# numericalEFT/FeynmanDiagram.jl

Measured on AMD Instinct MI355X. Metric: graph-evaluations/sec, higher is better.
Workload: dtype f64

## Files before the change

feynmandiagram.jl_amd/capi.py:

```python
from __future__ import annotations

import ctypes as C
import os
from typing import Optional

import numpy as np

from .nodetable import NodeTable

_HERE = os.path.dirname(os.path.abspath(__file__))
LIB_PATH = os.environ.get("FDG_LIBRARY") or os.path.join(_HERE, "lib", "libfdg.so")
KERNEL_CACHE = os.path.join(_HERE, "kernel_cache")

FDG_OK = 0
FDG_E_INVALID, FDG_E_UNSUPPORTED, FDG_E_NO_DEVICE, FDG_E_NOMEM, FDG_E_JIT, FDG_E_INTERNAL = -1, -2, -3, -4, -5, -6
FDG_SPEC_DEFAULT, FDG_SPEC_KEEP_SOURCE, FDG_SPEC_FAST_MATH, FDG_SPEC_ISA, FDG_SPEC_AUTOTUNE = 0, 1, 2, 4, 8
FDG_DT_F64, FDG_DT_F32, FDG_DT_C64, FDG_DT_C32 = 0, 1, 2, 3
DTYPES = {"Float64": FDG_DT_F64, "Float32": FDG_DT_F32, "ComplexF64": FDG_DT_C64, "ComplexF32": FDG_DT_C32}
FDG_SPEC_ROW_MAJOR_COMPANION = 16
FDG_ASSOC_STATIC, FDG_ASSOC_INTERP = 0, 1
FDG_TILE_SAMPLES = 64

EXPORTS = [
    "fdg_last_error", "fdg_version", "fdg_graph_create", "fdg_graph_destroy", "fdg_graph_query",
    "fdg_graph_emit_source", "fdg_free", "fdg_graph_specialize", "fdg_eval_device", "fdg_eval",
    "fdg_accumulate_device", "fdg_fill_uniform_device", "fdg_copy_device", "fdg_read_device", "fdg_clock_probe_device", "fdg_graph_specialize_typed", "fdg_eval_device_typed", "fdg_graph_create_complex_view", "fdg_isa_check_hazards", "fdg_graph_release_device", "fdg_powi",
    "fdg_eval_strided", "fdg_graph_coop_program", "fdg_graph_set_opt_params", "fdg_graph_opt_program", "fdg_graph_set_schedule_groups", "fdg_leaf_eval_device", "fdg_leaf_eval_device_tiled",
    "fdg_comm_unique_id", "fdg_comm_create", "fdg_comm_destroy", "fdg_reduce_device",
    "fdg_graph_specialize_fused", "fdg_mc_eval_device", "fdg_mc_accumulate_device", "fdg_graph_mc_program",
    "fdg_graph_kernel_info",
    "fdg_eval_device_tiled", "fdg_accumulate_device_tiled", "fdg_fill_uniform_device_tiled", "fdg_graph_set_association",
    "fdg_batch_alloc", "fdg_batch_free", "fdg_graph_pool_program", "fdg_batch_alloc_pair", "fdg_graph_set_option", "fdg_graph_get_option", "fdg_set_default_option", "fdg_get_default_option", "fdg_selftest_pair_search",
    "fdg_repack_tile_major", "fdg_unpack_tile_major",
    "fdg_accumulate_device_binned", "fdg_mc_accumulate_device_binned",
    "fdg_accumulate_device_moments", "fdg_mc_accumulate_device_moments",
    "fdg_vegas_sample_device", "fdg_accumulate_device_vegas", "fdg_mc_accumulate_device_vegas", "fdg_vegas_refine",
    "fdg_vegas_sample_device_discrete", "fdg_accumulate_device_vegas_binned", "fdg_mc_accumulate_device_vegas_binned",
    "fdg_vegas_refine_discrete",
    "fdg_vegas_sample_device_polar", "fdg_sincos",
    "fdg_matsubara_phase", "fdg_accumulate_device_matsubara", "fdg_mc_accumulate_device_matsubara",
    "fdg_vegas_sample_device_grouped", "fdg_accumulate_device_grouped", "fdg_mc_accumulate_device_grouped",
    "fdg_accumulate_device_observables", "fdg_mc_accumulate_device_observables",
    "fdg_accumulate_device_freq_observables", "fdg_mc_accumulate_device_freq_observables",
    "fdg_vegas_sample_device_strat", "fdg_accumulate_device_strat", "fdg_mc_accumulate_device_strat", "fdg_strat_allocate",
    "fdg_vegas_sample_device_strat_grouped", "fdg_accumulate_device_strat_grouped", "fdg_mc_accumulate_device_strat_grouped",
    "fdg_strat_allocate_cols",
    "fdg_chain_propose_device", "fdg_chain_step_device", "fdg_mc_chain_step_device", "fdg_chain_reduce_device",
# ... 142 lines not shown
    L.fdg_free.argtypes = [vp]
    L.fdg_free.restype = None
    L.fdg_graph_specialize.argtypes = [vp, C.c_char_p, C.c_uint]
    L.fdg_eval_device.argtypes = [vp, dp, i64, i64, dp, i64, i64, i64, vp]
    L.fdg_eval.argtypes = [vp, dp, dp, i64]
    L.fdg_graph_set_association.argtypes = [vp, C.c_int]
    L.fdg_batch_alloc.argtypes = [C.c_size_t, C.c_size_t, C.POINTER(vp)]
    L.fdg_batch_free.argtypes = [vp]
    L.fdg_graph_set_option.argtypes = [vp, C.c_char_p, C.c_char_p]
    L.fdg_graph_get_option.argtypes = [vp, C.c_char_p]
    L.fdg_graph_get_option.restype = C.c_char_p
    L.fdg_set_default_option.argtypes = [C.c_char_p, C.c_char_p]
    L.fdg_get_default_option.argtypes = [C.c_char_p]
    L.fdg_get_default_option.restype = C.c_char_p
    L.fdg_selftest_pair_search.argtypes = [C.c_uint64, C.c_uint32, C.c_uint32, C.POINTER(C.c_uint32)]
    L.fdg_batch_alloc_pair.argtypes = [vp, C.c_int64, C.c_size_t, C.c_uint, C.POINTER(vp), C.POINTER(vp), C.POINTER(BatchPairInfo)]
    L.fdg_eval_device_tiled.argtypes = [vp, dp, i64, i64, i64, dp, i64, i64, i64, i64, vp]
    L.fdg_accumulate_device_tiled.argtypes = [vp, dp, i64, i64, i64, dp, dp, i64, vp]
    L.fdg_fill_uniform_device_tiled.argtypes = [dp, i64, u32, i64, i64, i64, u64, u64, vp]
    L.fdg_eval_strided.argtypes = [vp, dp, i64, i64, dp, i64, i64, i64]
    L.fdg_accumulate_device.argtypes = [vp, dp, i64, i64, dp, dp, i64, vp]
    L.fdg_fill_uniform_device.argtypes = [dp, i64, u32, i64, i64, u64, u64, vp]
    L.fdg_copy_device.argtypes = [dp, dp, i64, vp]
    L.fdg_read_device.argtypes = [dp, i64, dp, vp]
    L.fdg_repack_tile_major.argtypes = [dp, i64, i64, dp, i64, C.c_uint32, vp]
    L.fdg_unpack_tile_major.argtypes = [dp, dp, i64, i64, i64, C.c_uint32, vp]
    L.fdg_clock_probe_device.argtypes = [C.c_double, vp, vp]
    L.fdg_graph_specialize_typed.argtypes = [vp, C.c_int, C.c_char_p, C.c_uint]
    L.fdg_eval_device_typed.argtypes = [vp, C.c_int, vp, i64, i64, vp, i64, i64, i64, vp]
    L.fdg_graph_create_complex_view.argtypes = [vp, C.POINTER(vp)]
# ... 1693 lines not shown
```

feynmandiagram.jl_amd/csrc/fdg_internal.h:

```cpp
#pragma once
#include <cstdint>
#include <mutex>
#include <string>
#include <vector>

#include "../../include/fdg.h"
#include "fdg_knobs.h"

namespace fdg {

constexpr uint32_t SP_LDS = 0u, SP_MEM = 1u, SP_LEAF = 2u;
constexpr uint32_t LOC_FAC = 1u << 29;
constexpr uint32_t LOC_IDX_MASK = (1u << 29) - 1u;
inline uint32_t mkloc(uint32_t space, uint32_t idx) { return (space << 30) | idx; }

constexpr uint32_t UOP_SUM = 0, UOP_PROD = 1, UOP_POW = 2, UOP_ROOT = 3, UOP_LEAF = 4, UOP_END = 5, UOP_PRODI = 6;

struct Lowered {
  uint32_t L = 0, N = 0, R = 0, E = 0;
  std::vector<uint8_t> op;
  std::vector<int32_t> power;
  std::vector<uint32_t> off, idx;
  std::vector<double> fac;
  std::vector<uint32_t> root_slot;
// ... 37 lines not shown
  void *s2 = nullptr, *ev_t[2] = {nullptr, nullptr}, *ev_k[2] = {nullptr, nullptr}, *ev_in = nullptr;
  uint64_t last_use = 0;
};

struct fdg_launch_cfg {
  bool no_rl = false, no_fused_acc = false, no_pool = false, pool_no_acc = false, no_streaming = false, no_w2 = false, no_coop = false, no_rm = false;
  bool transpose_narrow = false;
  uint32_t root_scratch_min = 16;
  uint64_t root_scratch_mb = 256;
  int waves_per_cu = 0;
  int oversub = 0;
  long mem_waves = -1;
  long mem_oversub = 1;
  double mem_ratio = 2.5;
  int tile_claim = -1;
  uint64_t sm_chunk_bytes = 1ull << 29;
  long long eval_chunk = 0, mc_chunk = 0;
};

enum { FDG_K_EVAL = 0, FDG_K_NT, FDG_K_W2, FDG_K_ACC, FDG_K_ACC_NT, FDG_K_RM, FDG_K_RM_ACC, FDG_K_RL, FDG_K_RL_ACC, FDG_K_COOP, FDG_K_POOL, FDG_K_EVAL_CL, FDG_K_NT_CL, FDG_K_COUNT };
static const char *const FDG_ISA_KERNEL[FDG_K_COUNT] = {"fdg_isa_eval", "fdg_isa_eval_nt", "fdg_isa_eval_w2", "fdg_isa_eval_acc", "fdg_isa_eval_acc_nt",
    "fdg_isa_eval_rm", "fdg_isa_eval_rm_acc", "fdg_isa_eval_rl", "fdg_isa_eval_rl_acc", "fdg_isa_eval_coop", "fdg_isa_eval_pool", "fdg_isa_eval_cl", "fdg_isa_eval_nt_cl"};
inline const char *fdg_isa_suffix(int k) { return FDG_ISA_KERNEL[k] + sizeof("fdg_isa_eval") - 1; }
struct fdg_isa_kernel {
  bool present = false;
  void *fn = nullptr;
  uint32_t vgpr = 0, lds_bytes = 0, mem_slots = 0, threads = 64;
};

struct fdg_graph {
// ... 11 lines not shown
  unsigned spec_flags = 0;
  uint32_t spec_vgpr = 0, spec_lds = 0, spec_scratch = 0;
  std::mutex mu;
  void *d_code = nullptr;
  void *d_root_live = nullptr;
  void *d_ws = nullptr;
  size_t ws_bytes = 0;
  void *module = nullptr;
  void *fn_eval_sm = nullptr, *fn_eval_gen = nullptr;
  bool isa = false;
  bool isa_fma = false;
  fdg_isa_kernel kern[FDG_K_COUNT];
  uint64_t st_valu[3] = {0, 0, 0};
  uint32_t st_ld_leaf[3] = {0, 0, 0}, st_panel[3] = {0, 0, 0}, st_lds[3] = {0, 0, 0};
  const char *last_kernel = "";
  uint32_t claim_run = 0;
  uint32_t last_launch = 0;
  uint32_t rm_bufs = 0;
  uint64_t rl_valu = 0;
  bool coop_enabled = false;
  uint32_t coop_panel_wg = 0;
  uint32_t pool_panel_wg = 0, pool_fetch = 0, pool_unit = 1;
  uint64_t pool_valu = 0;
  std::vector<char> alt_code;
  void *alt_module = nullptr, *fn_alt_sm = nullptr, *fn_alt_gen = nullptr;
  std::vector<char> fused_code;
  void *fused_module = nullptr, *fn_fused = nullptr;
  std::vector<char> typed_code[4];
  void *typed_module[4] = {nullptr, nullptr, nullptr, nullptr}, *fn_typed[4] = {nullptr, nullptr, nullptr, nullptr};
  fdg_graph *cx_twin = nullptr;
  bool cx_twin_tried = false;
// ... 84 lines not shown
```

feynmandiagram.jl_amd/csrc/fdg_isa.cpp:

```cpp
#include <algorithm>
#include <cctype>
#include <cinttypes>
#include <cmath>
#include <cstdio>
#include <cstdlib>
#include <cstring>
#include <map>
#include <sstream>

#include "fdg_opt.h"

namespace fdg {
int isa_claim_run_log2() {
  const char *e = fdg::knob("FDG_ISA_CLAIM_RUN");
  const long tiles = e ? std::atol(e) : 4;
  int r = 0;
  while (r < 6 && (1l << (r + 1)) <= tiles) ++r;
  return r;
}
namespace {

constexpr int V_LANE8 = 1, V_LEAFOFF = 2, V_ROOTOFF = 3, V_TMP = 4, V_BASE = 6;
constexpr int S_LEAF = 4, S_SS = 6, S_LS = 8, S_ROOT = 10, S_RS = 12, S_RK = 14, S_WS = 16, S_B = 18, S_NWG = 20;
constexpr int S_TILE = 22, S_NTILES = 23, S_LT = 24, S_RT = 26, S_PANEL = 28, S_LS8 = 30, S_RK8 = 32, S_A = 34,
              S_T = 36, S_C = 38, S_X = 40;
constexpr int S_WGT = 44;
constexpr int S_RTS = 44;
constexpr int S_LTS = 46;
constexpr int S_LP = 48;
constexpr int S_DELTA = 50;
constexpr int N_DELTA = 6;
constexpr int S_POOL = S_DELTA + 2 * N_DELTA;
constexpr int N_POOL = 20;
// ... 466 lines not shown
  const bool use_ldexp = fdg::knob("FDG_ISA_NO_LDEXP") == nullptr;
  const bool dbg_novalu = dbg && std::strstr(dbg, "novalu");
  const bool dbg_nopanel = dbg && std::strstr(dbg, "nopanel");
  const bool dbg_norecv = dbg && std::strstr(dbg, "norecv");
  const bool dbg_nofetch = dbg && std::strstr(dbg, "nopoolfetch");
  const bool dbg_noacc = dbg && std::strstr(dbg, "noacc");
  const bool dbg_nohead = dbg && std::strstr(dbg, "nohead");
  bool in_head = true;
  int tile_run = 0;
  if (dbg && std::strstr(dbg, "chunk") && !cs) tile_run = std::max(0, std::min(9, std::atoi(std::strstr(dbg, "chunk") + 5)));
  const bool tile_xcd = dbg && std::strstr(dbg, "xcd") && !cs && !tile_run;
  int tile_rot = 0;
  if (dbg && std::strstr(dbg, "rot") && !cs && !tile_run && !tile_xcd) tile_rot = std::max(0, std::atoi(std::strstr(dbg, "rot") + 3));
  const int S_ROTB = S_POOL + 2 * (N_POOL - 1), S_ROTS = S_ROTB + 1;
  const bool claim = claim_tiles && W == 1 && !cs && !accumulate && !rm_bufs && !rl && prog.mc_n_k == 0 && prog.mc_n_t == 0 && !tile_run && !tile_xcd && !tile_rot;
  const int claim_run = claim ? isa_claim_run_log2() : 0;
  const int S_CLAIM = S_POOL + 2 * (N_POOL - 1);
  uint64_t claim_seq = 0;
  E.vm_slack = (dbg && std::strstr(dbg, "noackwait") && !accumulate) ? p.R : 0;
  E.no_vm_wait = dbg && std::strstr(dbg, "novmwait");
  if (cs) E.ins("v_and_b32_e32 v0, 63, v0");
  E.ins("s_load_dwordx8 s[4:11], s[0:1], 0x0");
  E.ins("s_load_dwordx8 s[12:19], s[0:1], 0x20");
  E.ins("s_load_dwordx2 s[20:21], s[0:1], 0x40");
  if (accumulate) E.ins("s_load_dwordx2 " + S2(S_WGT) + ", s[0:1], 0x48");
  const uint32_t n_k = prog.mc_n_k;
  const bool mc = n_k > 0 || prog.mc_n_t > 0;
  const bool tm_imm = dbg && std::strstr(dbg, "tmimm") && !mc && !rm_bufs && !rl && !cs && W == 1;
  int64_t tm_base = -1;
  const int tile_arg = mc ? 0x80 : 0x50;
  E.ins("s_load_dwordx2 " + S2(S_LTS) + ", s[0:1], " + hex32((uint32_t)tile_arg));
  if (!accumulate) E.ins("s_load_dwordx2 " + S2(S_RTS) + ", s[0:1], " + hex32((uint32_t)tile_arg + 8));
  if (claim) E.ins("s_load_dwordx2 " + S2(S_CLAIM) + ", s[0:1], " + hex32((uint32_t)tile_arg + 16));
  if (mc) {
    E.ins("s_load_dwordx4 s[" + std::to_string(S_LEAF2) + ":" + std::to_string(S_LEAF2 + 3) + "], s[0:1], 0x50");
    E.ins("s_load_dwordx8 s[" + std::to_string(S_PARAM) + ":" + std::to_string(S_PARAM + 7) + "], s[0:1], 0x60");
  }
  E.ins("s_waitcnt lgkmcnt(0)");
  uint64_t w_seq = 0;
  const uint32_t acc0 = V_BASE + RW * std::max<uint32_t>(prog.n_reg_used, 1);
  const bool aa = accumulate && prog.params.acc_in_agpr;
  const uint32_t A0 = RW * prog.n_acc_used;
  const uint32_t acc_pairs_v = accumulate ? (aa ? 3 : p.R + 2) : 0;
  const uint32_t wgt0 = aa ? acc0 : acc0 + 2 * p.R;
  auto vpair = [&](uint32_t b) { return "v[" + std::to_string(b) + ":" + std::to_string(b + 1) + "]"; };
  auto vacc = [&](uint32_t k) { return vpair(acc0 + 2 * k); };
  const std::string vwgt = vpair(wgt0), vtmp = vpair(wgt0 + 2), vtmp2 = vpair(wgt0 + 4);
  auto acc_to_tmp2 = [&](uint32_t k) {
// ... 123 lines not shown
  E.ins("s_add_u32 " + S(S_X) + ", " + S(S_B) + ", " + std::to_string((1 << TSH) - 1));
  E.ins("s_addc_u32 " + S(S_X + 1) + ", " + S(S_B + 1) + ", 0");
  E.ins("s_lshr_b64 " + S2(S_X) + ", " + S2(S_X) + ", " + std::to_string(TSH));
  E.ins("s_mov_b32 " + S(S_NTILES) + ", " + S(S_X));
  if (tile_run) E.ins("s_lshl_b32 " + S(S_TILE) + ", s2, " + std::to_string(tile_run));
  else if (tile_xcd) {
    E.ins("s_and_b32 " + S(S_X) + ", s2, 7");
    E.ins("s_add_u32 " + S(S_T) + ", " + S(S_NTILES) + ", 7");
    E.ins("s_lshr_b32 " + S(S_T) + ", " + S(S_T) + ", 3");
    E.ins("s_mul_i32 " + S(S_A) + ", " + S(S_X) + ", " + S(S_T));
    E.ins("s_lshr_b32 " + S(S_A + 1) + ", s2, 3");
    E.ins("s_add_u32 " + S(S_TILE) + ", " + S(S_A) + ", " + S(S_A + 1));
    E.ins("s_add_u32 " + S(S_A) + ", " + S(S_A) + ", " + S(S_T));
    E.ins("s_min_u32 " + S(S_NTILES) + ", " + S(S_A) + ", " + S(S_NTILES));
  }
  else if (claim_run) E.ins("s_lshl_b32 " + S(S_TILE) + ", s2, " + std::to_string(claim_run));
  else {
    E.ins("s_mov_b32 " + S(S_TILE) + ", s2");
    if (tile_rot) { E.ins("s_mov_b32 " + S(S_ROTB) + ", 0"); E.ins("s_mov_b32 " + S(S_ROTS) + ", s2"); }
  }
  E.ins("s_mul_i32 " + S(S_X) + ", s2, " + hex32(cs ? cs->panel_wg_bytes : panel_bytes_per_wave));
  E.ins("s_mul_hi_u32 " + S(S_X + 1) + ", s2, " + hex32(cs ? cs->panel_wg_bytes : panel_bytes_per_wave));
  E.ins("s_add_u32 " + S(S_PANEL) + ", " + S(S_WS) + ", " + S(S_X));
  E.ins("s_addc_u32 " + S(S_PANEL + 1) + ", " + S(S_WS + 1) + ", " + S(S_X + 1));
  if (cs && cs->panel_prefix_bytes) {
    E.ins("s_add_u32 " + S(S_PANEL) + ", " + S(S_PANEL) + ", " + hex32(cs->panel_prefix_bytes));
    E.ins("s_addc_u32 " + S(S_PANEL + 1) + ", " + S(S_PANEL + 1) + ", 0");
  }
  std::map<uint32_t, int> panel_base;
  if (!mc) {
    std::map<uint32_t, uint64_t> hist;
// ... 8 lines not shown
    std::sort(v.begin(), v.end(), [](const auto &x, const auto &y) { return x.first > y.first || (x.first == y.first && x.second < y.second); });
    for (size_t i = 0; i < v.size() && pool.size() + i < (size_t)(N_POOL - (claim ? 1 : 0)); ++i) {
      const int r = S_POOL + 2 * (int)(pool.size() + i);
      panel_base[v[i].second] = r;
      E.ins("s_add_u32 " + S(r) + ", " + S(S_PANEL) + ", " + hex32(v[i].second * 8192u));
      E.ins("s_addc_u32 " + S(r + 1) + ", " + S(S_PANEL + 1) + ", 0");
    }
  }
  E.ins("s_cmp_ge_u32 " + S(S_TILE) + ", " + S(S_NTILES));
  E.ins("s_cbranch_scc0 .Ltile" + sfx);
  E.ins("s_endpgm");
  os << ".Ltile" << sfx << ":\n";
  if (cs && cs->slack) E.ins("s_mov_b32 " + S(S_DELTA + 7) + ", " + S(S_DELTA + 6));
  const int v_claim = (int)(tmp0 + 2 * n_tmp_pairs);
  if (claim) {
    if (claim_run) {
      E.ins("s_and_b32 " + S(S_X) + ", " + S(S_TILE) + ", " + std::to_string((1 << claim_run) - 1));
      E.ins("s_cbranch_scc1 .Lheld" + sfx);
    }
    E.ins("s_mov_b64 exec, 1");
    E.ins("v_mov_b32_e32 " + V(V_TMP) + ", 1");
    E.ins("global_atomic_add " + V(v_claim) + ", " + V(V_LANE8) + ", " + V(V_TMP) + ", " + S2(S_CLAIM) + " sc0");
    if (claim_run) os << ".Lheld" << sfx << ":\n";
    claim_seq = ++E.vm_issued;
  }
  E.ins("s_mov_b32 " + S(S_X + 1) + ", 0");
  E.ins("s_mov_b32 " + S(S_X) + ", " + S(S_TILE));
  E.ins("s_lshl_b64 " + S2(S_X) + ", " + S2(S_X) + ", " + std::to_string(TSH));
  if (W == 1) {
    E.ins("s_sub_u32 " + S(S_T) + ", " + S(S_B) + ", " + S(S_X));
    E.ins("s_subb_u32 " + S(S_T + 1) + ", " + S(S_B + 1) + ", " + S(S_X + 1));
    E.ins("s_cmp_lg_u32 " + S(S_T + 1) + ", 0");
    E.ins("s_cselect_b32 " + S(S_T) + ", 64, " + S(S_T));
    E.ins("s_min_u32 " + S(S_T) + ", " + S(S_T) + ", 64");
    E.ins("s_bfm_b64 " + S2(S_A) + ", " + S(S_T) + ", 0");
    E.ins("s_cmp_ge_u32 " + S(S_T) + ", 64");
    E.ins("s_cselect_b64 exec, -1, " + S2(S_A));
  }
// ... 553 lines not shown
    E.ins("s_cbranch_scc1 .Lrun" + sfx);
    E.ins("s_lshl_b32 " + S(S_X) + ", " + S(S_NWG) + ", " + std::to_string(tile_run));
    E.ins("s_add_u32 " + S(S_TILE) + ", " + S(S_TILE) + ", " + S(S_X));
    E.ins("s_sub_u32 " + S(S_TILE) + ", " + S(S_TILE) + ", " + std::to_string(1 << tile_run));
    os << ".Lrun" << sfx << ":\n";
  } else if (tile_xcd) {
    E.ins("s_lshr_b32 " + S(S_X) + ", " + S(S_NWG) + ", 3");
    E.ins("s_add_u32 " + S(S_TILE) + ", " + S(S_TILE) + ", " + S(S_X));
  } else if (tile_rot) {
    E.ins("s_add_u32 " + S(S_ROTB) + ", " + S(S_ROTB) + ", " + S(S_NWG));
    E.ins("s_add_u32 " + S(S_ROTS) + ", " + S(S_ROTS) + ", " + std::to_string(tile_rot));
    E.ins("s_sub_u32 " + S(S_X) + ", " + S(S_NWG) + ", 1");
    E.ins("s_and_b32 " + S(S_ROTS) + ", " + S(S_ROTS) + ", " + S(S_X));
    E.ins("s_add_u32 " + S(S_TILE) + ", " + S(S_ROTB) + ", " + S(S_ROTS));
  } else if (claim) {
    if (claim_run) {
      E.ins("s_add_u32 " + S(S_TILE) + ", " + S(S_TILE) + ", 1");
      E.ins("s_and_b32 " + S(S_X) + ", " + S(S_TILE) + ", " + std::to_string((1 << claim_run) - 1));
      E.ins("s_cbranch_scc1 .Lrun" + sfx);
    }
    if (claim_seq > E.vm_done) {
      const uint64_t n = std::min<uint64_t>(E.vm_issued - claim_seq, 63);
      E.ins("s_waitcnt vmcnt(" + std::to_string(n) + ")");
      E.vm_done = std::max(std::max(E.vm_done, E.vm_issued - n), claim_seq);
    }
    E.ins("v_readfirstlane_b32 " + S(S_TILE) + ", " + V(v_claim));
    E.ins("s_add_u32 " + S(S_TILE) + ", " + S(S_TILE) + ", " + S(S_NWG));
    if (claim_run) {
      E.ins("s_lshl_b32 " + S(S_TILE) + ", " + S(S_TILE) + ", " + std::to_string(claim_run));
      os << ".Lrun" << sfx << ":\n";
    }
  } else {
    E.ins("s_add_u32 " + S(S_TILE) + ", " + S(S_TILE) + ", " + S(S_NWG));
  }
  E.ins("s_cmp_ge_u32 " + S(S_TILE) + ", " + S(S_NTILES));
  E.ins("s_cbranch_scc0 .Lback" + sfx);
  if (accumulate) {
    E.ins("s_mov_b64 exec, -1");
    E.ins("v_lshlrev_b32_e32 " + V(V_TMP) + ", 2, v0");
    if (aa)
      for (uint32_t k = 0; k < p.R; ++k) {
        acc_to_tmp2(k);
        for (int off = 32; off >= 1; off >>= 1) {
          E.ins("v_xor_b32_e32 " + V(V_TMP + 1) + ", " + std::to_string(off * 4) + ", " + V(V_TMP));
          E.ins("ds_bpermute_b32 v" + std::to_string(wgt0 + 2) + ", " + V(V_TMP + 1) + ", v" + std::to_string(wgt0 + 4));
          E.ins("ds_bpermute_b32 v" + std::to_string(wgt0 + 3) + ", " + V(V_TMP + 1) + ", v" + std::to_string(wgt0 + 5));
// ... 28 lines not shown
  E.ins("s_endpgm");
  os << ".Lback" << sfx << ":\n";
  E.ins("s_getpc_b64 " + S2(S_A));
  os << ".Lpc" << sfx << ":\n";
  E.ins("s_add_u32 " + S(S_A) + ", " + S(S_A) + ", (.Ltile" + sfx + "-.Lpc" + sfx + ")&0xffffffff");
  E.ins("s_addc_u32 " + S(S_A + 1) + ", " + S(S_A + 1) + ", (.Ltile" + sfx + "-.Lpc" + sfx + ")>>32");
  E.ins("s_setpc_b64 " + S2(S_A));
  E.ins("s_endpgm");

  const uint32_t next_vgpr = std::max<uint32_t>(V_BASE + RW * std::max<uint32_t>(prog.n_reg_used, 1) + 2 * acc_pairs_v + 2 * n_tmp_pairs + (rm_bufs ? 10 : 0) + (cs ? (cs->slack ? 7 : 4) : 0) + (rl ? 2 : 0) + (claim ? 1 : 0), 8);
  const uint32_t accum = (next_vgpr + 3) & ~3u;
  const uint32_t n_agpr = RW * prog.n_acc_used + (aa ? 2 * p.R : 0);
  if (cs) return KernelMeta{kname, lds_bytes, accum, n_agpr, 12, (mc || has_macro) ? S_END : S_POOL + 2 * 16};
  os << "\t.section\t.rodata,\"a\",@progbits\n\t.p2align\t6, 0x0\n\t.amdhsa_kernel " << kname << "\n";
  os << "\t\t.amdhsa_group_segment_fixed_size " << lds_bytes << "\n";
  os << "\t\t.amdhsa_private_segment_fixed_size 0\n\t\t.amdhsa_kernarg_size " << (mc ? 144 : (claim ? 104 : 96)) << "\n\t\t.amdhsa_user_sgpr_count 2\n";
  os << "\t\t.amdhsa_user_sgpr_kernarg_segment_ptr 1\n\t\t.amdhsa_system_sgpr_workgroup_id_x 1\n";
  os << "\t\t.amdhsa_system_vgpr_workitem_id 0\n";
  const int n_sgpr = (mc || has_macro || claim) ? S_END : S_POOL + 2 * 16;
  os << "\t\t.amdhsa_next_free_vgpr " << (accum + n_agpr) << "\n\t\t.amdhsa_next_free_sgpr " << n_sgpr << "\n";
  os << "\t\t.amdhsa_accum_offset " << accum << "\n\t\t.amdhsa_reserve_vcc 1\n";
  os << "\t\t.amdhsa_float_round_mode_32 0\n\t\t.amdhsa_float_round_mode_16_64 0\n";
  os << "\t\t.amdhsa_float_denorm_mode_32 3\n\t\t.amdhsa_float_denorm_mode_16_64 3\n";
  os << "\t\t.amdhsa_dx10_clamp 1\n\t\t.amdhsa_ieee_mode 1\n";
  os << "\t.end_amdhsa_kernel\n";
  (void)p;
  return KernelMeta{kname, lds_bytes, accum, n_agpr, mc ? 18 : (claim ? 13 : 12), n_sgpr};
}

}

static KernelMeta emit_coop(Emit &E, const Lowered &p, const CoopProgram &cp, const std::string &kname) {
  std::ostringstream &os = E.os;
  os << "\t.text\n\t.protected\t" << kname << "\n\t.globl\t" << kname << "\n\t.p2align\t8\n\t.type\t" << kname << ",@function\n";
  os << kname << ":\n";
  E.off = 0;
  E.klabel = kname;
  const char *ca = fdg::knob("FDG_COOP_ALIGN");
  E.pad_ok = ca ? ca[0] == '1' : cp.pooled;
  const int align_before = E.align;
  if (cp.pooled && !ca && E.align == 1) E.align = 2;
  E.hz.reset();
// ... 125 lines not shown
    ks.push_back(emit_kernel(E, p, prog, kname + "_cl", 1, false, 0, nullptr, false, true));
    if (!fdg::knob("FDG_ISA_NO_STREAMING")) {
      E.streaming = true;
      ks.push_back(emit_kernel(E, p, prog, kname + "_nt_cl", 1, false, 0, nullptr, false, true));
      E.streaming = false;
    }
  }
  std::ostringstream &os = E.os;
  os << "\t.text\n\t.amdgpu_metadata\n---\namdhsa.kernels:\n";
  const char *kinds[18] = {"global_buffer", "by_value", "by_value", "global_buffer", "by_value", "by_value",
                           "global_buffer", "by_value", "by_value", "global_buffer", "global_buffer", "by_value",
                           "by_value", "by_value", "by_value", "by_value", "by_value", "by_value"};
  for (const KernelMeta &k : ks) {
    os << "  - .agpr_count: " << k.n_agpr << "\n    .args:\n";
    for (int i = 0; i < k.n_args; ++i) {
      const char *kind = (k.n_args <= 13 && i >= 10) ? (i == 12 ? "global_buffer" : "by_value") : kinds[i];
      os << "      - .offset: " << i * 8 << "\n        .size: 8\n        .value_kind: " << kind << "\n";
      if (std::strcmp(kind, "global_buffer") == 0) os << "        .address_space: global\n";
    }
    os << "    .group_segment_fixed_size: " << k.lds_bytes << "\n    .kernarg_segment_align: 8\n    .kernarg_segment_size: " << 8 * k.n_args << "\n";
    os << "    .max_flat_workgroup_size: " << k.wg << "\n    .name: " << k.name << "\n    .private_segment_fixed_size: 0\n";
    os << "    .sgpr_count: " << (k.n_sgpr + 6) << "\n    .sgpr_spill_count: 0\n    .symbol: " << k.name << ".kd\n";
    os << "    .uniform_work_group_size: 1\n    .uses_dynamic_stack: false\n    .vgpr_count: " << (k.accum + k.n_agpr)
       << "\n    .vgpr_spill_count: 0\n    .wavefront_size: 64\n";
  }
  if (records) for (const KernelMeta &k : ks) records->push_back(IsaKernelRecord{k.name, k.accum + k.n_agpr, k.lds_bytes, k.wg});
  os << "amdhsa.target: amdgcn-amd-amdhsa--gfx950\namdhsa.version:\n  - 1\n  - 2\n...\n\t.end_amdgpu_metadata\n";
  return os.str();
}

}
// ... 1 lines not shown
```

feynmandiagram.jl_amd/csrc/fdg_opt.h:

```cpp
#pragma once
#include <cstdint>
#include <string>
#include <vector>

#include "fdg_internal.h"

namespace fdg {

enum MKind : uint8_t {
  M_LD_LEAF = 0,
  M_LD_LDS,
  M_LD_MEM,
  M_ST_LDS,
  M_ST_MEM,
  M_MUL,
  M_ADD,
  M_MULC,
  M_ROOT,
  M_MOV,
  M_LD_ACC,
  M_ST_ACC,
  M_FMA = 14,
  M_FMAC = 15,
  M_ADDC = 16,
// ... 102 lines not shown
  CoopProgram coop, pool;
  bool w2 = false, acc = false, rm_acc = false, rl = false, rl_acc = false;
  uint32_t rm_bufs = 0;
  int coop_verdict = -1;
  const OptProgram *w2_prog() const { return w2 ? &p2 : nullptr; }
  const OptProgram *acc_prog() const { return acc ? &pa : nullptr; }
  const OptProgram *rm_prog() const { return rm_bufs ? &pr : nullptr; }
  const OptProgram *rm_acc_prog() const { return rm_bufs && rm_acc ? &pra : nullptr; }
  const OptProgram *rl_prog() const { return rl ? &prl : nullptr; }
  const OptProgram *rl_acc_prog() const { return rl && rl_acc ? &prla : nullptr; }
  const CoopProgram *coop_prog() const { return coop.supported ? &coop : nullptr; }
  const CoopProgram *pool_prog() const { return pool.supported ? &pool : nullptr; }
};
struct IsaKernelRecord { std::string name; uint32_t vgpr = 0 , lds_bytes = 0, threads = 64; };
std::string emit_isa(const Lowered &p, const IsaPrograms &V, std::vector<IsaKernelRecord> *records = nullptr);
int isa_claim_run_log2();

void rm_plan_stats(const Lowered &p, const OptProgram &prog, uint32_t bufs, uint64_t &fetches, uint64_t &gathers);
int check_isa_hazards(const std::string &text, std::string &report);
std::string isa_hazard_table();

}
```

feynmandiagram.jl_amd/csrc/fdg_runtime.hip:

```cpp
#include <hip/hip_runtime.h>
#include <hip/hiprtc.h>
#include <fcntl.h>
#include <sys/stat.h>
#include <sys/wait.h>
#include <unistd.h>

#include <atomic>
#include <cstdio>
#include <cstdlib>
#include <cstring>
#include <fstream>
#include <sstream>

#define FDG_RUNTIME_TU 1
#include "fdg_internal.h"
#include "fdg_opt.h"
#include "fdg_powi.h"

using namespace fdg;


typedef const __attribute__((address_space(4))) uint32_t cword;

__device__ __forceinline__ double fdg_block_sum256(double v, double *sh) {
// ... 543 lines not shown
  c.no_pool = get("FDG_ISA_NO_POOL") != nullptr;
  c.pool_no_acc = get("FDG_ISA_POOL_NO_ACC") != nullptr;
  c.no_streaming = get("FDG_ISA_NO_STREAMING") != nullptr;
  c.no_w2 = get("FDG_ISA_NO_W2") != nullptr;
  c.no_coop = get("FDG_ISA_NO_COOP") != nullptr;
  c.no_rm = get("FDG_ISA_NO_RM") != nullptr;
  c.transpose_narrow = get("FDG_TRANSPOSE_NARROW") != nullptr;
  if (const char *e = get("FDG_ROOT_SCRATCH_MIN")) c.root_scratch_min = (uint32_t)std::max(0, std::atoi(e));
  if (const char *e = get("FDG_ROOT_SCRATCH_MB")) c.root_scratch_mb = (uint64_t)std::max(1, std::atoi(e));
  if (const char *e = get("FDG_ISA_WAVES_PER_CU")) c.waves_per_cu = std::max(1, std::atoi(e));
  if (const char *e = get("FDG_ISA_OVERSUB")) c.oversub = std::max(1, std::atoi(e));
  if (const char *e = get("FDG_ISA_MEM_WAVES")) c.mem_waves = std::max(0l, std::atol(e));
  if (const char *e = get("FDG_ISA_MEM_OVERSUB")) c.mem_oversub = std::max(1l, std::atol(e));
  if (const char *e = get("FDG_ISA_MEM_RATIO")) c.mem_ratio = std::atof(e);
  if (const char *e = get("FDG_ISA_TILE_CLAIM")) c.tile_claim = e[0] != '0' ? 1 : 0;
  if (const char *e = get("FDG_SM_CHUNK_MB")) c.sm_chunk_bytes = (uint64_t)std::max(1, std::atoi(e)) << 20;
  if (const char *e = get("FDG_EVAL_CHUNK")) c.eval_chunk = std::atoll(e);
  if (const char *e = get("FDG_MC_CHUNK")) c.mc_chunk = std::atoll(e);
  g->cfg = c;
}

static int run(fdg_graph *g, int mode, const double *d_leaf, int64_t ss, int64_t ls, double *d_root,
               int64_t rs, int64_t rk, const double *d_weight, double *d_acc, int64_t B, hipStream_t st,
               int64_t lts = 0, int64_t rts = 0) {
  if (!g) { set_error("null handle"); return FDG_E_INVALID; }
  if (B < 0) { set_error("n_sample < 0"); return FDG_E_INVALID; }
  if (B == 0) return FDG_OK;
  if ((g->prog.L && !d_leaf) || (mode == 0 && g->prog.R && !d_root) || (mode == 1 && !d_acc)) {
    set_error("null device buffer"); return FDG_E_INVALID;
  }
  if (mode == 1 && g->prog.R == 0) return FDG_OK;
  std::lock_guard<std::mutex> lk(g->mu);
  fdg::KnobScope knob_scope(&g->knobs);
  { const int rcb = fdg_bind_stream_ws(g, (void *)st); if (rcb) return rcb; }
// ... 127 lines not shown
  hipLaunchKernelGGL(fdg_reduce_lane_partials, dim3(std::min<uint32_t>(R, 64u)), dim3(256), 0, st, part, nwg, R, acc);
  HIP_TRY(hipGetLastError());
  return FDG_OK;
}

struct IsaRun {
  fdg_graph *g;
  const RunArgs &a;
  const Lowered &p;
  const uint32_t R;
  const bool tiled;
  long ntiles = 0, grid = 0, grid_cl = 0, grid2 = 0, grid3 = 0, grid4 = 0, grid5 = 0;
  size_t panel_all = 0;
  bool pool_ok = false, fused_acc = false, wide_ss = false, named = false, claim = false;
  size_t claim_off = 0;
  double *roots = nullptr;
  long a_rs = 0, a_rk = 0;

  IsaRun(fdg_graph *g_, const RunArgs &a_) : g(g_), a(a_), p(g_->prog), R(g_->prog.R), tiled(a_.lts != 0 || a_.rts != 0) {}

  const fdg_isa_kernel &K(int k) const { return g->kern[k]; }
  uint32_t waves_per_cu(const fdg_isa_kernel &k) const {
    return g->cfg.waves_per_cu > 0 ? (uint32_t)g->cfg.waves_per_cu : isa_waves_per_cu(k.vgpr, k.lds_bytes);
  }
  long oversub(long resident, size_t bytes_per_wg) const {
    if (g->cfg.waves_per_cu > 0) return resident;
    long f = g->cfg.oversub > 0 ? g->cfg.oversub : 8;
    while (f > 1 && (ntiles < resident * f * 4 || bytes_per_wg * (size_t)(resident * f) > ((size_t)32 << 20))) f >>= 1;
    return resident * f;
  }
// ... 41 lines not shown
    int rc = ensure_ws(g, claim_off + 256);
    if (rc) return rc;
    roots = a.d_root; a_rs = (long)a.rs; a_rk = (long)a.rk;
    if (a.mode == 1 && !fused_acc) {
      rc = ensure_root_scratch(g, (size_t)((a.B + 15) & ~(int64_t)15) * std::max<uint32_t>(R, 1) * sizeof(double) + (size_t)2048 * R * sizeof(double));
      if (rc) return rc;
      roots = (double *)g->d_ws2; a_rs = 1; a_rk = (long)((a.B + 15) & ~(int64_t)15);
    }
    wide_ss = a.ss < 0 || a.ss >= (1ll << 23);
    return FDG_OK;
  }

  int launch(int k, const double *lf, long lss, long lls, double *rt, long rrs, long rrk, long n, long nwg, const double *wt, long tls, long trs) {
    void *a_wsp = g->d_ws;
    void *a_cnt = (char *)g->d_ws + claim_off;
    void *args[] = {(void *)&lf, &lss, &lls, (void *)&rt, &rrs, &rrk, &a_wsp, &n, &nwg, (void *)&wt, &tls, &trs, &a_cnt};
    if (k == FDG_K_EVAL_CL || k == FDG_K_NT_CL) HIP_TRY(hipMemsetAsync(a_cnt, 0, 4, a.st));
    HIP_TRY(hipModuleLaunchKernel((hipFunction_t)K(k).fn, (unsigned)nwg, 1, 1, K(k).threads, 1, 1, 0, a.st, args, nullptr));
    g->last_launch = (uint32_t)nwg | ((k == FDG_K_EVAL_CL || k == FDG_K_NT_CL) ? FDG_LAUNCH_CLAIMED : 0u);
    return FDG_OK;
  }
  int launch_reduced(int k, const double *lf, long lss, long lls, double *part, long n, long nwg, const double *wt, long tls) {
    const int rc = launch(k, lf, lss, lls, part, 0, 0, n, nwg, wt, tls, 0);
    return rc ? rc : launch_reduce_lane_partials(part, (uint32_t)nwg, R, a.d_acc, a.st);
  }
  int launch_acc(const double *lf, long lss, long lls, const double *wt, long n, long tls = 0) {
    double *part = (double *)((char *)g->d_ws + panel_all);
    if (!tls) tls = 64 * lss;
    const int k = K(FDG_K_ACC_NT).fn && line_aligned(lf, lss, lls) && (tls & 15) == 0 ? FDG_K_ACC_NT : FDG_K_ACC;
    if (!named) g->last_kernel = FDG_ISA_KERNEL[k];
    return launch_reduced(k, lf, lss, lls, part, n, std::min<long>((n + 63) / 64, grid3), wt, tls);
// ... 3 lines not shown
    if (K(FDG_K_W2).present && lss == 1 && n >= 128 && !tls && !trs && !g->cfg.no_w2) {
      const long n2 = n & ~127l;
      const int rc = launch(FDG_K_W2, lf, lss, lls, rt, rrs, rrk, n2, std::min<long>(n2 / 128, grid2), nullptr, 128 * lss, 128 * rrs);
      if (rc) return rc;
      g->last_kernel = FDG_ISA_KERNEL[FDG_K_W2];
      done = n2;
    }
    if (done < n) {
      const double *lf1 = lf + done * lss;
      double *rt1 = rt + done * rrs;
      const long n1 = n - done;
      if (!tls) tls = 64 * lss;
      if (!trs) trs = 64 * rrs;
      int k = K(FDG_K_NT).fn && line_aligned(lf1, lss, lls) && line_aligned(rt1, rrs, rrk) && ((tls | trs) & 15) == 0 ? FDG_K_NT : FDG_K_EVAL;
      if (!named && done == 0) g->last_kernel = FDG_ISA_KERNEL[k];
      long run = 1, nwg = grid;
      if (claim && (g->cfg.tile_claim > 0 || (n1 + 63) / 64 >= 256 * grid) && K(k == FDG_K_NT ? FDG_K_NT_CL : FDG_K_EVAL_CL).fn) { k = k == FDG_K_NT ? FDG_K_NT_CL : FDG_K_EVAL_CL; run = 1l << g->claim_run; nwg = grid_cl; }
      return launch(k, lf1, lss, lls, rt1, rrs, rrk, n1, std::min<long>(((n1 + 63) / 64 + run - 1) / run, nwg), nullptr, tls, trs);
    }
    return FDG_OK;
  }
  int finish_scratch_acc() {
    double *partial = roots + (size_t)a_rk * R;
    const uint32_t pb = weighted_segments((long)a.B, R);
    const uint8_t *live = nullptr;
    const int rcl = root_live_mask(g, &live);
    if (rcl) return rcl;
    hipLaunchKernelGGL(fdg_weighted_partials, dim3(pb * R), dim3(256), 0, a.st, roots, a_rk, a.d_weight, (long)a.B, R, pb, partial, live);
    hipLaunchKernelGGL(fdg_reduce_partials, dim3(std::min<uint32_t>(R, 64u)), dim3(256), 0, a.st, partial, pb, R, a.d_acc);
    HIP_TRY(hipGetLastError());
    return FDG_OK;
  }

// ... 707 lines not shown
}

static void install_isa(fdg_graph *g, const fdg::IsaPrograms &V, std::vector<char> &co, const std::string &hash, unsigned flags,
                        const std::vector<fdg::IsaKernelRecord> &records) {
  if (g->module) { hipModuleUnload((hipModule_t)g->module); g->module = nullptr; }
  fill_isa_kernels(g->kern, V, records);
  const fdg_isa_kernel *K = g->kern;
  if (K[FDG_K_RL].present) g->rl_valu = V.prl.n_valu;
  if (K[FDG_K_POOL].present) {
    g->pool_panel_wg = panel_bytes_per_wg(V.pool);
    g->pool_fetch = (uint32_t)V.pool.n_transfer;
    g->pool_unit = V.pool.pool_unit;
    g->pool_valu = 0;
    for (uint32_t w = 0; w < V.pool.n_wave; ++w) g->pool_valu += V.pool.wave[w].n_valu;
  }
  g->claim_run = (uint32_t)fdg::isa_claim_run_log2();
  g->coop_enabled = K[FDG_K_COOP].present;
  if (K[FDG_K_COOP].present) g->coop_panel_wg = panel_bytes_per_wg(V.coop);
  g->code_object.swap(co);
  g->isa = true;
  g->spec_vgpr = K[FDG_K_EVAL].vgpr; g->spec_lds = K[FDG_K_EVAL].lds_bytes; g->spec_scratch = 0;
  const fdg::OptProgram *pp[3] = {V.main, V.acc_prog(), V.rm_prog()};
  for (int i = 0; i < 3; ++i) {
    g->st_valu[i] = pp[i] ? pp[i]->n_valu : 0;
    g->st_ld_leaf[i] = pp[i] ? (uint32_t)pp[i]->n_ld_leaf : 0;
    g->st_panel[i] = pp[i] ? (uint32_t)(pp[i]->n_ld_mem + pp[i]->n_st_mem) : 0;
    g->st_lds[i] = pp[i] ? (uint32_t)(pp[i]->n_ld_lds + pp[i]->n_st_lds) : 0;
  }
  g->rm_bufs = V.rm_bufs;
  g->last_kernel = "";
  g->spec_source_hash = hash;
// ... 1010 lines not shown
```

include/fdg.h:

```cpp
#ifndef FDG_H
#define FDG_H

#include <stddef.h>
#include <stdint.h>

#ifdef __cplusplus
extern "C" {
#endif

#define FDG_VERSION 102

#define FDG_OP_SUM 0u
#define FDG_OP_PROD 1u
#define FDG_OP_POWER 2u
#define FDG_NO_ROOT 0xFFFFFFFFu

enum {
  FDG_OK = 0,
  FDG_E_INVALID = -1,
  FDG_E_UNSUPPORTED = -2,
  FDG_E_NO_DEVICE = -3,
  FDG_E_NOMEM = -4,
  FDG_E_JIT = -5,
  FDG_E_INTERNAL = -6
// ... 167 lines not shown
  uint32_t n_filler;
  uint32_t n_probe;
  uint32_t n_matched;
  uint32_t calibrated;
  double gbs_fast, gbs_slow;
  double gbs_before_mean, gbs_before_min;
  double gbs_after_mean, gbs_after_min;
  double seconds;
  double seconds_settling;
  uint32_t level_reached;
  uint32_t span_gb;
} fdg_batch_pair_info;
int fdg_batch_alloc_pair(fdg_graph *g, int64_t n_sample, size_t chunk_bytes_hint, unsigned flags, void **d_leaf, void **d_root,
                         fdg_batch_pair_info *info);
int fdg_selftest_pair_search(uint64_t seed, uint32_t scenario, uint32_t n_window, uint32_t *n_probe);

int fdg_fill_uniform_device(double *d_leaf, int64_t n_sample, uint32_t n_leaf,
                            int64_t leaf_sample_stride, int64_t leaf_leaf_stride, uint64_t seed,
                            uint64_t sample_offset, void *stream);

int fdg_isa_check_hazards(const char *asm_text, char **report);

int fdg_copy_device(double *d_dst, const double *d_src, int64_t n, void *stream);

int fdg_read_device(const double *d_src, int64_t n, double *d_sink, void *stream);

int fdg_clock_probe_device(double seconds, int64_t *d_ticks, void *stream);

typedef struct fdg_leaf_tables {
  uint32_t n_leaf, n_basis, n_loop, dim, n_tau;
// ... 313 lines not shown
```

Baseline: 9.935 billion.

## Pick atomic tile-claim run length at runtime from tile bytes and tile count

Result: no change. 9.930 billion (-0.1%).

```diff
diff --git a/feynmandiagram.jl_amd/capi.py b/feynmandiagram.jl_amd/capi.py
--- a/feynmandiagram.jl_amd/capi.py
+++ b/feynmandiagram.jl_amd/capi.py
@@ -30,7 +30,7 @@
     "fdg_graph_specialize_fused", "fdg_mc_eval_device", "fdg_mc_accumulate_device", "fdg_graph_mc_program",
     "fdg_graph_kernel_info",
     "fdg_eval_device_tiled", "fdg_accumulate_device_tiled", "fdg_fill_uniform_device_tiled", "fdg_graph_set_association",
-    "fdg_batch_alloc", "fdg_batch_free", "fdg_graph_pool_program", "fdg_batch_alloc_pair", "fdg_graph_set_option", "fdg_graph_get_option", "fdg_set_default_option", "fdg_get_default_option", "fdg_selftest_pair_search",
+    "fdg_batch_alloc", "fdg_batch_free", "fdg_graph_pool_program", "fdg_batch_alloc_pair", "fdg_graph_set_option", "fdg_graph_get_option", "fdg_set_default_option", "fdg_get_default_option", "fdg_selftest_pair_search", "fdg_selftest_claim_plan",
     "fdg_repack_tile_major", "fdg_unpack_tile_major",
     "fdg_accumulate_device_binned", "fdg_mc_accumulate_device_binned",
     "fdg_accumulate_device_moments", "fdg_mc_accumulate_device_moments",
@@ -203,6 +203,7 @@
     L.fdg_get_default_option.argtypes = [C.c_char_p]
     L.fdg_get_default_option.restype = C.c_char_p
     L.fdg_selftest_pair_search.argtypes = [C.c_uint64, C.c_uint32, C.c_uint32, C.POINTER(C.c_uint32)]
+    L.fdg_selftest_claim_plan.argtypes = [C.c_uint32, C.c_uint32, C.c_int64, C.c_int64, C.c_int64, C.c_int, C.c_int64, C.c_int64, C.c_int64, C.POINTER(C.c_uint32), C.POINTER(C.c_int64)]
     L.fdg_batch_alloc_pair.argtypes = [vp, C.c_int64, C.c_size_t, C.c_uint, C.POINTER(vp), C.POINTER(vp), C.POINTER(BatchPairInfo)]
     L.fdg_eval_device_tiled.argtypes = [vp, dp, i64, i64, i64, dp, i64, i64, i64, i64, vp]
     L.fdg_accumulate_device_tiled.argtypes = [vp, dp, i64, i64, i64, dp, dp, i64, vp]
diff --git a/feynmandiagram.jl_amd/csrc/fdg_internal.h b/feynmandiagram.jl_amd/csrc/fdg_internal.h
--- a/feynmandiagram.jl_amd/csrc/fdg_internal.h
+++ b/feynmandiagram.jl_amd/csrc/fdg_internal.h
@@ -75,6 +75,9 @@
   long mem_oversub = 1;
   double mem_ratio = 2.5;
   int tile_claim = -1;
+  long claim_run = 0;
+  long claim_bytes = 128l << 10;
+  long claim_min_runs = 0;
   uint64_t sm_chunk_bytes = 1ull << 29;
   long long eval_chunk = 0, mc_chunk = 0;
 };
@@ -116,7 +119,6 @@
   uint64_t st_valu[3] = {0, 0, 0};
   uint32_t st_ld_leaf[3] = {0, 0, 0}, st_panel[3] = {0, 0, 0}, st_lds[3] = {0, 0, 0};
   const char *last_kernel = "";
-  uint32_t claim_run = 0;
   uint32_t last_launch = 0;
   uint32_t rm_bufs = 0;
   uint64_t rl_valu = 0;
diff --git a/feynmandiagram.jl_amd/csrc/fdg_isa.cpp b/feynmandiagram.jl_amd/csrc/fdg_isa.cpp
--- a/feynmandiagram.jl_amd/csrc/fdg_isa.cpp
+++ b/feynmandiagram.jl_amd/csrc/fdg_isa.cpp
@@ -11,12 +11,29 @@
 #include "fdg_opt.h"
 
 namespace fdg {
-int isa_claim_run_log2() {
-  const char *e = fdg::knob("FDG_ISA_CLAIM_RUN");
-  const long tiles = e ? std::atol(e) : 4;
+int isa_claim_run_log2(long tiles) {
   int r = 0;
   while (r < 6 && (1l << (r + 1)) <= tiles) ++r;
   return r;
+}
+
+ClaimPlan isa_claim_plan(uint32_t n_leaf, uint32_t n_root, long ntiles, long grid, long grid_cl, int tile_claim, long claim_run, long claim_bytes, long min_runs) {
+  ClaimPlan c;
+  if (min_runs <= 0) min_runs = n_leaf >= 24 ? 64 : 128;
+  if (tile_claim == 0 || grid <= 0 || grid_cl <= 0 || ntiles <= 0) return c;
+  int run = -1;
+  if (claim_run > 0) run = isa_claim_run_log2(claim_run);
+  else if (tile_claim > 0) run = 2;
+  else {
+    const long tile_bytes = 512l * ((long)n_leaf + (long)n_root);
+    for (int r = 0; r <= 6 && run < 0; ++r) if ((tile_bytes << r) >= claim_bytes) run = r;
+    if (run < 0) return c;
+  }
+  if (tile_claim < 0 && min_runs > 1 && ntiles < ((min_runs * grid) << run)) return c;
+  c.claim = true;
+  c.run_log2 = run;
+  c.nwg = std::min<long>((ntiles + (1l << run) - 1) >> run, grid_cl);
+  return c;
 }
 namespace {
 
@@ -513,8 +530,7 @@
   if (dbg && std::strstr(dbg, "rot") && !cs && !tile_run && !tile_xcd) tile_rot = std::max(0, std::atoi(std::strstr(dbg, "rot") + 3));
   const int S_ROTB = S_POOL + 2 * (N_POOL - 1), S_ROTS = S_ROTB + 1;
   const bool claim = claim_tiles && W == 1 && !cs && !accumulate && !rm_bufs && !rl && prog.mc_n_k == 0 && prog.mc_n_t == 0 && !tile_run && !tile_xcd && !tile_rot;
-  const int claim_run = claim ? isa_claim_run_log2() : 0;
-  const int S_CLAIM = S_POOL + 2 * (N_POOL - 1);
+  const int S_CLAIM = S_POOL + 2 * (N_POOL - 1), S_RUN = 0;
   uint64_t claim_seq = 0;
   E.vm_slack = (dbg && std::strstr(dbg, "noackwait") && !accumulate) ? p.R : 0;
   E.no_vm_wait = dbg && std::strstr(dbg, "novmwait");
@@ -530,7 +546,11 @@
   const int tile_arg = mc ? 0x80 : 0x50;
   E.ins("s_load_dwordx2 " + S2(S_LTS) + ", s[0:1], " + hex32((uint32_t)tile_arg));
   if (!accumulate) E.ins("s_load_dwordx2 " + S2(S_RTS) + ", s[0:1], " + hex32((uint32_t)tile_arg + 8));
-  if (claim) E.ins("s_load_dwordx2 " + S2(S_CLAIM) + ", s[0:1], " + hex32((uint32_t)tile_arg + 16));
+  if (claim) {
+    E.ins("s_load_dwordx2 " + S2(S_CLAIM) + ", s[0:1], " + hex32((uint32_t)tile_arg + 16));
+    E.ins("s_load_dwordx2 " + S2(S_RUN) + ", s[0:1], " + hex32((uint32_t)tile_arg + 24));
+    for (int i = 0; i < 30; ++i) E.ins("s_nop 0");
+  }
   if (mc) {
     E.ins("s_load_dwordx4 s[" + std::to_string(S_LEAF2) + ":" + std::to_string(S_LEAF2 + 3) + "], s[0:1], 0x50");
     E.ins("s_load_dwordx8 s[" + std::to_string(S_PARAM) + ":" + std::to_string(S_PARAM + 7) + "], s[0:1], 0x60");
@@ -684,7 +704,7 @@
     E.ins("s_add_u32 " + S(S_A) + ", " + S(S_A) + ", " + S(S_T));
     E.ins("s_min_u32 " + S(S_NTILES) + ", " + S(S_A) + ", " + S(S_NTILES));
   }
-  else if (claim_run) E.ins("s_lshl_b32 " + S(S_TILE) + ", s2, " + std::to_string(claim_run));
+  else if (claim) E.ins("s_lshl_b32 " + S(S_TILE) + ", s2, " + S(S_RUN));
   else {
     E.ins("s_mov_b32 " + S(S_TILE) + ", s2");
     if (tile_rot) { E.ins("s_mov_b32 " + S(S_ROTB) + ", 0"); E.ins("s_mov_b32 " + S(S_ROTS) + ", s2"); }
@@ -723,14 +743,12 @@
   if (cs && cs->slack) E.ins("s_mov_b32 " + S(S_DELTA + 7) + ", " + S(S_DELTA + 6));
   const int v_claim = (int)(tmp0 + 2 * n_tmp_pairs);
   if (claim) {
-    if (claim_run) {
-      E.ins("s_and_b32 " + S(S_X) + ", " + S(S_TILE) + ", " + std::to_string((1 << claim_run) - 1));
-      E.ins("s_cbranch_scc1 .Lheld" + sfx);
-    }
+    E.ins("s_bfe_u32 " + S(S_X) + ", " + S(S_TILE) + ", " + S(S_RUN + 1));
+    E.ins("s_cbranch_scc1 .Lheld" + sfx);
     E.ins("s_mov_b64 exec, 1");
     E.ins("v_mov_b32_e32 " + V(V_TMP) + ", 1");
     E.ins("global_atomic_add " + V(v_claim) + ", " + V(V_LANE8) + ", " + V(V_TMP) + ", " + S2(S_CLAIM) + " sc0");
-    if (claim_run) os << ".Lheld" << sfx << ":\n";
+    os << ".Lheld" << sfx << ":\n";
     claim_seq = ++E.vm_issued;
   }
   E.ins("s_mov_b32 " + S(S_X + 1) + ", 0");
@@ -1314,11 +1332,9 @@
     E.ins("s_and_b32 " + S(S_ROTS) + ", " + S(S_ROTS) + ", " + S(S_X));
     E.ins("s_add_u32 " + S(S_TILE) + ", " + S(S_ROTB) + ", " + S(S_ROTS));
   } else if (claim) {
-    if (claim_run) {
-      E.ins("s_add_u32 " + S(S_TILE) + ", " + S(S_TILE) + ", 1");
-      E.ins("s_and_b32 " + S(S_X) + ", " + S(S_TILE) + ", " + std::to_string((1 << claim_run) - 1));
-      E.ins("s_cbranch_scc1 .Lrun" + sfx);
-    }
+    E.ins("s_add_u32 " + S(S_TILE) + ", " + S(S_TILE) + ", 1");
+    E.ins("s_bfe_u32 " + S(S_X) + ", " + S(S_TILE) + ", " + S(S_RUN + 1));
+    E.ins("s_cbranch_scc1 .Lrun" + sfx);
     if (claim_seq > E.vm_done) {
       const uint64_t n = std::min<uint64_t>(E.vm_issued - claim_seq, 63);
       E.ins("s_waitcnt vmcnt(" + std::to_string(n) + ")");
@@ -1326,10 +1342,8 @@
     }
     E.ins("v_readfirstlane_b32 " + S(S_TILE) + ", " + V(v_claim));
     E.ins("s_add_u32 " + S(S_TILE) + ", " + S(S_TILE) + ", " + S(S_NWG));
-    if (claim_run) {
-      E.ins("s_lshl_b32 " + S(S_TILE) + ", " + S(S_TILE) + ", " + std::to_string(claim_run));
-      os << ".Lrun" << sfx << ":\n";
-    }
+    E.ins("s_lshl_b32 " + S(S_TILE) + ", " + S(S_TILE) + ", " + S(S_RUN));
+    os << ".Lrun" << sfx << ":\n";
   } else {
     E.ins("s_add_u32 " + S(S_TILE) + ", " + S(S_TILE) + ", " + S(S_NWG));
   }
@@ -1388,7 +1402,7 @@
   if (cs) return KernelMeta{kname, lds_bytes, accum, n_agpr, 12, (mc || has_macro) ? S_END : S_POOL + 2 * 16};
   os << "\t.section\t.rodata,\"a\",@progbits\n\t.p2align\t6, 0x0\n\t.amdhsa_kernel " << kname << "\n";
   os << "\t\t.amdhsa_group_segment_fixed_size " << lds_bytes << "\n";
-  os << "\t\t.amdhsa_private_segment_fixed_size 0\n\t\t.amdhsa_kernarg_size " << (mc ? 144 : (claim ? 104 : 96)) << "\n\t\t.amdhsa_user_sgpr_count 2\n";
+  os << "\t\t.amdhsa_private_segment_fixed_size 0\n\t\t.amdhsa_kernarg_size " << (mc ? 144 : (claim ? 112 : 96)) << "\n\t\t.amdhsa_user_sgpr_count 2\n";
   os << "\t\t.amdhsa_user_sgpr_kernarg_segment_ptr 1\n\t\t.amdhsa_system_sgpr_workgroup_id_x 1\n";
   os << "\t\t.amdhsa_system_vgpr_workitem_id 0\n";
   const int n_sgpr = (mc || has_macro || claim) ? S_END : S_POOL + 2 * 16;
@@ -1399,7 +1413,7 @@
   os << "\t\t.amdhsa_dx10_clamp 1\n\t\t.amdhsa_ieee_mode 1\n";
   os << "\t.end_amdhsa_kernel\n";
   (void)p;
-  return KernelMeta{kname, lds_bytes, accum, n_agpr, mc ? 18 : (claim ? 13 : 12), n_sgpr};
+  return KernelMeta{kname, lds_bytes, accum, n_agpr, mc ? 18 : (claim ? 14 : 12), n_sgpr};
 }
 
 }
@@ -1555,7 +1569,7 @@
   for (const KernelMeta &k : ks) {
     os << "  - .agpr_count: " << k.n_agpr << "\n    .args:\n";
     for (int i = 0; i < k.n_args; ++i) {
-      const char *kind = (k.n_args <= 13 && i >= 10) ? (i == 12 ? "global_buffer" : "by_value") : kinds[i];
+      const char *kind = (k.n_args <= 14 && i >= 10) ? (i == 12 ? "global_buffer" : "by_value") : kinds[i];
       os << "      - .offset: " << i * 8 << "\n        .size: 8\n        .value_kind: " << kind << "\n";
       if (std::strcmp(kind, "global_buffer") == 0) os << "        .address_space: global\n";
     }
diff --git a/feynmandiagram.jl_amd/csrc/fdg_opt.h b/feynmandiagram.jl_amd/csrc/fdg_opt.h
--- a/feynmandiagram.jl_amd/csrc/fdg_opt.h
+++ b/feynmandiagram.jl_amd/csrc/fdg_opt.h
@@ -140,7 +140,9 @@
 };
 struct IsaKernelRecord { std::string name; uint32_t vgpr = 0 , lds_bytes = 0, threads = 64; };
 std::string emit_isa(const Lowered &p, const IsaPrograms &V, std::vector<IsaKernelRecord> *records = nullptr);
-int isa_claim_run_log2();
+int isa_claim_run_log2(long tiles);
+struct ClaimPlan { bool claim = false; int run_log2 = 0; long nwg = 0; };
+ClaimPlan isa_claim_plan(uint32_t n_leaf, uint32_t n_root, long ntiles, long grid, long grid_cl, int tile_claim, long claim_run, long claim_bytes, long min_runs);
 
 void rm_plan_stats(const Lowered &p, const OptProgram &prog, uint32_t bufs, uint64_t &fetches, uint64_t &gathers);
 int check_isa_hazards(const std::string &text, std::string &report);
diff --git a/feynmandiagram.jl_amd/csrc/fdg_runtime.hip b/feynmandiagram.jl_amd/csrc/fdg_runtime.hip
--- a/feynmandiagram.jl_amd/csrc/fdg_runtime.hip
+++ b/feynmandiagram.jl_amd/csrc/fdg_runtime.hip
@@ -581,10 +581,23 @@
   if (const char *e = get("FDG_ISA_MEM_OVERSUB")) c.mem_oversub = std::max(1l, std::atol(e));
   if (const char *e = get("FDG_ISA_MEM_RATIO")) c.mem_ratio = std::atof(e);
   if (const char *e = get("FDG_ISA_TILE_CLAIM")) c.tile_claim = e[0] != '0' ? 1 : 0;
+  if (const char *e = get("FDG_ISA_CLAIM_RUN")) c.claim_run = std::max(1l, std::atol(e));
+  if (const char *e = get("FDG_ISA_CLAIM_BYTES")) c.claim_bytes = std::max(1l, std::atol(e));
+  if (const char *e = get("FDG_ISA_CLAIM_MIN_RUNS")) c.claim_min_runs = std::max(1l, std::atol(e));
   if (const char *e = get("FDG_SM_CHUNK_MB")) c.sm_chunk_bytes = (uint64_t)std::max(1, std::atoi(e)) << 20;
   if (const char *e = get("FDG_EVAL_CHUNK")) c.eval_chunk = std::atoll(e);
   if (const char *e = get("FDG_MC_CHUNK")) c.mc_chunk = std::atoll(e);
   g->cfg = c;
+}
+
+int fdg_selftest_claim_plan(uint32_t n_leaf, uint32_t n_root, int64_t n_tile, int64_t grid, int64_t grid_cl, int tile_claim, int64_t claim_run,
+                            int64_t claim_bytes, int64_t min_runs, uint32_t *run, int64_t *n_wg) {
+  const fdg_launch_cfg d;
+  const fdg::ClaimPlan c = fdg::isa_claim_plan(n_leaf, n_root, (long)n_tile, (long)grid, (long)grid_cl, tile_claim, (long)claim_run,
+                                               claim_bytes > 0 ? (long)claim_bytes : d.claim_bytes, min_runs > 0 ? (long)min_runs : d.claim_min_runs);
+  if (run) *run = c.claim ? 1u << c.run_log2 : 0u;
+  if (n_wg) *n_wg = c.claim ? c.nwg : 0;
+  return c.claim ? 1 : 0;
 }
 
 static int run(fdg_graph *g, int mode, const double *d_leaf, int64_t ss, int64_t ls, double *d_root,
@@ -742,6 +755,7 @@
   size_t panel_all = 0;
   bool pool_ok = false, fused_acc = false, wide_ss = false, named = false, claim = false;
   size_t claim_off = 0;
+  uint32_t claim_run = 0;
   double *roots = nullptr;
   long a_rs = 0, a_rk = 0;
 
@@ -813,7 +827,8 @@
   int launch(int k, const double *lf, long lss, long lls, double *rt, long rrs, long rrk, long n, long nwg, const double *wt, long tls, long trs) {
     void *a_wsp = g->d_ws;
     void *a_cnt = (char *)g->d_ws + claim_off;
-    void *args[] = {(void *)&lf, &lss, &lls, (void *)&rt, &rrs, &rrk, &a_wsp, &n, &nwg, (void *)&wt, &tls, &trs, &a_cnt};
+    uint64_t a_run = (uint64_t)claim_run | ((uint64_t)claim_run << 48);
+    void *args[] = {(void *)&lf, &lss, &lls, (void *)&rt, &rrs, &rrk, &a_wsp, &n, &nwg, (void *)&wt, &tls, &trs, &a_cnt, &a_run};
     if (k == FDG_K_EVAL_CL || k == FDG_K_NT_CL) HIP_TRY(hipMemsetAsync(a_cnt, 0, 4, a.st));
     HIP_TRY(hipModuleLaunchKernel((hipFunction_t)K(k).fn, (unsigned)nwg, 1, 1, K(k).threads, 1, 1, 0, a.st, args, nullptr));
     g->last_launch = (uint32_t)nwg | ((k == FDG_K_EVAL_CL || k == FDG_K_NT_CL) ? FDG_LAUNCH_CLAIMED : 0u);
@@ -847,9 +862,13 @@
       if (!trs) trs = 64 * rrs;
       int k = K(FDG_K_NT).fn && line_aligned(lf1, lss, lls) && line_aligned(rt1, rrs, rrk) && ((tls | trs) & 15) == 0 ? FDG_K_NT : FDG_K_EVAL;
       if (!named && done == 0) g->last_kernel = FDG_ISA_KERNEL[k];
-      long run = 1, nwg = grid;
-      if (claim && (g->cfg.tile_claim > 0 || (n1 + 63) / 64 >= 256 * grid) && K(k == FDG_K_NT ? FDG_K_NT_CL : FDG_K_EVAL_CL).fn) { k = k == FDG_K_NT ? FDG_K_NT_CL : FDG_K_EVAL_CL; run = 1l << g->claim_run; nwg = grid_cl; }
-      return launch(k, lf1, lss, lls, rt1, rrs, rrk, n1, std::min<long>(((n1 + 63) / 64 + run - 1) / run, nwg), nullptr, tls, trs);
+      const long nt1 = (n1 + 63) / 64;
+      long nwg = std::min<long>(nt1, grid);
+      if (claim && K(k == FDG_K_NT ? FDG_K_NT_CL : FDG_K_EVAL_CL).fn) {
+        const fdg::ClaimPlan c = fdg::isa_claim_plan(p.L, R, nt1, grid, grid_cl, g->cfg.tile_claim, g->cfg.claim_run, g->cfg.claim_bytes, g->cfg.claim_min_runs);
+        if (c.claim) { k = k == FDG_K_NT ? FDG_K_NT_CL : FDG_K_EVAL_CL; claim_run = (uint32_t)c.run_log2; nwg = c.nwg; }
+      }
+      return launch(k, lf1, lss, lls, rt1, rrs, rrk, n1, nwg, nullptr, tls, trs);
     }
     return FDG_OK;
   }
@@ -1587,7 +1606,6 @@
     g->pool_valu = 0;
     for (uint32_t w = 0; w < V.pool.n_wave; ++w) g->pool_valu += V.pool.wave[w].n_valu;
   }
-  g->claim_run = (uint32_t)fdg::isa_claim_run_log2();
   g->coop_enabled = K[FDG_K_COOP].present;
   if (K[FDG_K_COOP].present) g->coop_panel_wg = panel_bytes_per_wg(V.coop);
   g->code_object.swap(co);
diff --git a/include/fdg.h b/include/fdg.h
--- a/include/fdg.h
+++ b/include/fdg.h
@@ -205,6 +205,8 @@
 int fdg_batch_alloc_pair(fdg_graph *g, int64_t n_sample, size_t chunk_bytes_hint, unsigned flags, void **d_leaf, void **d_root,
                          fdg_batch_pair_info *info);
 int fdg_selftest_pair_search(uint64_t seed, uint32_t scenario, uint32_t n_window, uint32_t *n_probe);
+int fdg_selftest_claim_plan(uint32_t n_leaf, uint32_t n_root, int64_t n_tile, int64_t grid, int64_t grid_cl, int tile_claim, int64_t claim_run,
+                            int64_t claim_bytes, int64_t min_runs, uint32_t *run, int64_t *n_wg);
 
 int fdg_fill_uniform_device(double *d_leaf, int64_t n_sample, uint32_t n_leaf,
                             int64_t leaf_sample_stride, int64_t leaf_leaf_stride, uint64_t seed,
```
